# guptakhil/show-tell

Hardware: AMD Instinct MI355X
Metric: training images/sec (ResNet101+GRU, emb=512, bs=128) at 1/2/4/8 MI355X (higher is better)
Workload: dtype bf16; 1 GPU; BASELINE configs[1]: ResNet-101 (train-mode BN, frozen) + 5-layer GRU decoder, E=H=512, V=10000, fwd+bwd+SGD step, synthetic COCO-shaped batch; batch_per_gpu=128, global_batch=128, image=3x224x224, parallelism=dp1

## Files before the change

### include/showtell_hip.h

```cpp
#ifndef SHOWTELL_HIP_H
#define SHOWTELL_HIP_H

#include <stddef.h>
#include <stdint.h>

#ifdef __cplusplus
extern "C" {
#endif

#define ST_F32 0
#define ST_BF16 1

#define ST_CELL_GRU 0
#define ST_CELL_LSTM 1

const char* st_last_error(void);
int st_version(void);

typedef struct {
  const void* x;
  const void* w;
  void* y;
  const float* bias;
  const float* scale;
// ... 168 lines not shown

int st_cast2d(const void* x, void* y, int from_dtype, int to_dtype, int rows, int cols, int ldx, int ldy, void* stream);

#define ST_MAX_LAYERS 8
typedef struct {
  int cell, dtype, L, in0, H, V, E;
  const void* emb;
  const void* w_ih[ST_MAX_LAYERS]; const void* w_hh[ST_MAX_LAYERS];
  const float* b_ih[ST_MAX_LAYERS]; const float* b_hh[ST_MAX_LAYERS];
  const void* w_lin; const float* b_lin;
} st_rnn_params;

typedef struct {
  float* emb;
  float* w_ih[ST_MAX_LAYERS]; float* w_hh[ST_MAX_LAYERS]; float* b_ih[ST_MAX_LAYERS]; float* b_hh[ST_MAX_LAYERS];
  float* w_lin; float* b_lin;
} st_rnn_grads;

typedef struct {
  int B, T, ntok, Tcap;
  const int* batch_sizes_host;
  const int* rows_b; const int* rows_t; const int* prev_row;
  const long* caption;
} st_packed_seq;

int st_rnn_vocab_ld(int V);
size_t st_rnn_workspace_bytes(const st_rnn_params* p, const st_packed_seq* s);
int st_rnn_forward(const st_rnn_params* p, const st_packed_seq* s, const void* x0_override, const void* feat,
                   void* workspace, size_t workspace_bytes, void* logits, int logits_dtype, int ldl,
                   long* targets, int save_for_backward, void* stream);
int st_rnn_backward(const st_rnn_params* p, const st_rnn_grads* g, const st_packed_seq* s,
                    const void* x0_override, const void* dlogits, int ldd, const float* dy_top,
                    void* workspace, size_t workspace_bytes, float* dfeat, float* dx0_out, void* stream);

int st_rnn_fused_loss_supported(const st_rnn_params* p);
size_t st_rnn_fused_loss_bytes(const st_rnn_params* p, const st_packed_seq* s);
int st_rnn_fused_loss(const st_rnn_params* p, const st_packed_seq* s, const void* workspace, size_t workspace_bytes,
                      const long* targets, float* scratch, size_t scratch_bytes, float* loss_accum, void* stream);
int st_rnn_fused_dlogits(const st_rnn_params* p, const st_packed_seq* s, const void* workspace, size_t workspace_bytes,
                         const long* targets, const float* scratch, const float* grad_scale_dev, void* dlogits, int ldd, void* stream);

int st_cross_entropy(const void* logits, int logits_dtype, const long* target, int rows, int V, int ldl,
                     float* loss_accum, void* dlogits, int dlogits_dtype, int ldd, float grad_scale,
                     const float* grad_scale_dev , void* stream);

size_t st_head_workspace_bytes(int B, int F, int E, int dtype);
int st_linear_bn1d_forward(const void* x, const void* w, const float* bias, const float* gamma, const float* beta,
                           float* running_mean, float* running_var, int B, int F, int E, int dtype,
                           int train, float momentum, float eps,
                           float* z_out, float* save_mean, float* save_rstd, void* y_dtype, float* y_f32, void* stream);
int st_linear_bn1d_backward(const float* dy, const float* z, const void* x, const float* gamma,
                            const float* save_mean, const float* save_rstd, int B, int F, int E, int dtype, int train,
                            float* dw, float* dbias, float* dgamma, float* dbeta, void* workspace, size_t workspace_bytes,
                            void* stream);

int st_sgd_step(float* param, const float* grad, float* momentum_buf, void* bf16_shadow, long n,
                float lr, float momentum, int first_step, float grad_scale, void* stream);
int st_adam_step(float* param, const float* grad, float* exp_avg, float* exp_avg_sq, void* bf16_shadow, long n,
                 float lr, float beta1, float beta2, float eps, int step, float grad_scale, void* stream);

size_t st_rnn_greedy_workspace_bytes(const st_rnn_params* p, int B);
int st_rnn_greedy(const st_rnn_params* p, const void* feat, int B, int steps, void* workspace, size_t workspace_bytes,
                  long* ids_out, float* logits_out, void* stream);
int st_rnn_greedy_last_route(void);

int st_rnn_step(const st_rnn_params* p, const void* x, int n, const void* h_in, const void* c_in,
// ... 47 lines not shown
```

### show-tell_amd/_lib.py

```python
import ctypes as C
import os

_HERE = os.path.dirname(os.path.abspath(__file__))
LIB_PATH = os.path.join(_HERE, "lib", "libshowtell_hip.so")

ST_F32, ST_BF16 = 0, 1
ST_CELL_GRU, ST_CELL_LSTM = 0, 1

c_p, c_i, c_f, c_l = C.c_void_p, C.c_int, C.c_float, C.c_long


class ConvDesc(C.Structure):
    _fields_ = [("x", c_p), ("w", c_p), ("y", c_p), ("bias", c_p), ("scale", c_p), ("shift", c_p),
                ("residual", c_p), ("stats", c_p), ("dtype", c_i), ("out_dtype", c_i),
                ("B", c_i), ("Hin", c_i), ("Win", c_i), ("Cin", c_i), ("Ho", c_i), ("Wo", c_i), ("N", c_i),
                ("KH", c_i), ("KW", c_i), ("stride", c_i), ("pad", c_i),
                ("ldx", c_i), ("ldw", c_i), ("ldy", c_i), ("relu", c_i), ("accumulate", c_i), ("Cin_logical", c_i), ("k_order", c_i), ("stats_replicas", c_i),
                ("in_stats", c_p), ("in_gamma", c_p), ("in_beta", c_p), ("in_count", c_f), ("in_eps", c_f), ("split_k", c_i)]


class Conv3x3ImgDesc(C.Structure):
    _fields_ = [("x", c_p), ("w_frag", c_p), ("y", c_p), ("stats", c_p), ("stats_replicas", c_i), ("scale", c_p), ("shift", c_p),
                ("relu", c_i), ("in_stats", c_p), ("in_gamma", c_p), ("in_beta", c_p), ("in_count", c_f), ("in_eps", c_f),
                ("B", c_i), ("H", c_i), ("W", c_i), ("C", c_i), ("N", c_i), ("in_stats_replicas", c_i)]
# ... 103 lines not shown
    "st_conv1x1_kstream": ([C.POINTER(Conv1x1WregDesc), c_p], c_i),
    "st_pack_conv_weight_frag": ([c_p, c_p, c_i, c_i, c_i, c_i, c_i, c_p], c_i),
    "st_tune": ([c_i, c_i, c_i], c_i),
    "st_prof_enable": ([c_i], c_i),
    "st_debug_stamps": ([c_p], c_i),
    "st_prof_collect": ([C.POINTER(C.c_double), C.POINTER(C.c_double), C.POINTER(c_l)], c_i),
    "st_bn_act": ([C.POINTER(BnActDesc), c_p], c_i),
    "st_bn_update_running": ([c_p, c_p, c_p, c_i, c_f, c_f, c_p], c_i),
    "st_nchw_to_nhwc": ([c_p, c_p, c_i, c_i, c_i, c_i, c_i, c_i, c_p], c_i),
    "st_nchw_to_s2d16": ([c_p, c_p, c_i, c_i, c_i, c_i, c_p], c_i),
    "st_stem_weight_s2d": ([c_p, c_p, c_i, c_i, c_p], c_i),
    "st_stem_weight_frag": ([c_p, c_p, c_p], c_i),
    "st_stem_weight_frag_packed": ([c_p, c_i, c_p, c_p], c_i),
    "st_stem_conv_pool": ([C.POINTER(StemConvPoolDesc), c_p], c_i),
    "st_nhwc_to_ncp_f32": ([c_p, c_p, c_i, c_i, c_i, c_i, c_p], c_i),
    "st_maxpool3x3s2": ([c_p, c_p, c_i, c_i, c_i, c_i, c_i, c_p], c_i),
    "st_maxpool3x3s2_bn": ([c_p, c_p, c_i, c_i, c_i, c_i, c_i, c_p, c_p, c_p, c_p, c_p, c_f, c_f, c_p], c_i),
    "st_global_avgpool": ([c_p, c_p, c_i, c_i, c_i, c_i, c_i, c_p], c_i),
    "st_cast": ([c_p, c_p, c_i, c_i, c_l, c_p], c_i),
    "st_transpose": ([c_p, c_p, c_i, c_i, c_i, c_i, c_i, c_p], c_i),
    "st_transpose_colsum": ([c_p, c_p, c_p, c_i, c_i, c_i, c_i, c_i, c_p], c_i),
    "st_transpose_batch": ([c_p, c_p, c_p, c_i, c_i, c_i, c_i, c_i, c_i, c_p, c_p, c_p], c_i),
    "st_pack_conv_weight": ([c_p, c_p, c_i, c_i, c_i, c_i, c_i, c_i, c_i, c_p], c_i),
    "st_cast2d": ([c_p, c_p, c_i, c_i, c_i, c_i, c_i, c_i, c_p], c_i),
    "st_rnn_vocab_ld": ([c_i], c_i),
    "st_rnn_workspace_bytes": ([C.POINTER(RnnParams), C.POINTER(PackedSeq)], C.c_size_t),
    "st_rnn_forward": ([C.POINTER(RnnParams), C.POINTER(PackedSeq), c_p, c_p, c_p, C.c_size_t, c_p, c_i, c_i, c_p, c_i, c_p], c_i),
    "st_rnn_fused_loss_supported": ([C.POINTER(RnnParams)], c_i),
    "st_rnn_fused_loss_bytes": ([C.POINTER(RnnParams), C.POINTER(PackedSeq)], C.c_size_t),
    "st_rnn_fused_loss": ([C.POINTER(RnnParams), C.POINTER(PackedSeq), c_p, C.c_size_t, c_p, c_p, C.c_size_t, c_p, c_p], c_i),
    "st_rnn_fused_dlogits": ([C.POINTER(RnnParams), C.POINTER(PackedSeq), c_p, C.c_size_t, c_p, c_p, c_p, c_p, c_i, c_p], c_i),
    "st_rnn_backward": ([C.POINTER(RnnParams), C.POINTER(RnnGrads), C.POINTER(PackedSeq), c_p, c_p, c_i, c_p, c_p, C.c_size_t,
                         c_p, c_p, c_p], c_i),
    "st_rnn_greedy_workspace_bytes": ([C.POINTER(RnnParams), c_i], C.c_size_t),
    "st_rnn_greedy": ([C.POINTER(RnnParams), c_p, c_i, c_i, c_p, C.c_size_t, c_p, c_p, c_p], c_i),
    "st_rnn_greedy_last_route": ([], c_i),
    "st_rnn_step": ([C.POINTER(RnnParams), c_p, c_i, c_p, c_p, c_p, c_p, c_p, c_i, c_p], c_i),
    "st_embedding_rows": ([c_p, c_p, c_p, c_i, c_i, c_i, c_i, c_i, c_p], c_i),
    "st_gather_state": ([c_p, c_p, c_p, c_i, c_i, c_i, c_i, c_i, c_p], c_i),
    "st_softmax_topk": ([c_p, c_i, c_i, c_i, c_i, c_p, c_p, c_i, c_p], c_i),
    "st_beam_select": ([c_p, c_p, c_p, c_p, c_p, c_i, c_i, c_i, c_l, c_p, c_p, c_p, c_p, c_p, c_p], c_i),
    "st_attn_workspace_bytes": ([c_p, c_p], C.c_size_t),
    "st_attn_forward": ([c_p, c_p, c_p, c_p, c_p, C.c_size_t, c_p, c_i, c_i, c_p, c_i, c_p], c_i),
    "st_attn_backward": ([c_p, c_p, c_p, c_p, c_p, c_i, c_p, c_p, c_f, c_p, c_p, C.c_size_t, c_p], c_i),
    "st_attn_reg_loss": ([c_p, c_i, c_i, c_i, c_f, c_p, c_p], c_i),
    "st_attn_greedy_workspace_bytes": ([c_p, c_i], C.c_size_t),
    "st_attn_greedy": ([c_p, c_p, c_i, c_i, c_l, c_p, C.c_size_t, c_p, c_p], c_i),
    "st_attn_greedy_alphas": ([c_p, c_p, c_i, c_i, c_l, c_p, C.c_size_t, c_p, c_p, c_p], c_i),
    "st_attn_beam_workspace_bytes": ([c_p, c_i, c_i], C.c_size_t),
    "st_attn_beam_search": ([c_p, c_p, c_i, c_i, c_i, c_l, c_l, c_p, C.c_size_t, c_p, c_p, c_p, c_p, c_p, c_p], c_i),
    "st_cross_entropy": ([c_p, c_i, c_p, c_i, c_i, c_i, c_p, c_p, c_i, c_i, c_f, c_p, c_p], c_i),
    "st_head_workspace_bytes": ([c_i, c_i, c_i, c_i], C.c_size_t),
    "st_linear_bn1d_forward": ([c_p] * 7 + [c_i, c_i, c_i, c_i, c_i, c_f, c_f] + [c_p] * 6, c_i),
    "st_linear_bn1d_backward": ([c_p] * 6 + [c_i, c_i, c_i, c_i, c_i] + [c_p] * 5 + [C.c_size_t, c_p], c_i),
    "st_sgd_step": ([c_p, c_p, c_p, c_p, c_l, c_f, c_f, c_i, c_f, c_p], c_i),
    "st_adam_step": ([c_p, c_p, c_p, c_p, c_p, c_l, c_f, c_f, c_f, c_f, c_i, c_f, c_p], c_i),
    "st_resnet_create": ([c_i, c_i, C.POINTER(c_p)], c_i),
    "st_resnet_destroy": ([c_p], None),
    "st_resnet_num_convs": ([c_p], c_i),
    "st_resnet_feat_dim": ([c_p], c_i),
    "st_resnet_weight_elems": ([c_p], C.c_size_t),
    "st_resnet_bn_channels": ([c_p], C.c_size_t),
    "st_resnet_conv_info": ([c_p, c_i] + [C.POINTER(c_i)] * 6 + [C.POINTER(C.c_size_t)] * 2 + [C.POINTER(c_i), C.POINTER(C.c_size_t), C.POINTER(c_i)], c_i),
    "st_resnet_workspace_bytes": ([c_p, c_i, c_i, c_i], C.c_size_t),
    "st_resnet_set_taps": ([c_p, c_p, C.c_size_t], c_i),
    "st_resnet_forward": ([c_p, c_p, c_i, c_i, c_i, c_p, c_p, c_p, c_p, c_p, c_i, c_f, c_f, c_p, C.c_size_t,
# ... 47 lines not shown
```

### show-tell_amd/csrc/rnn.cpp

```cpp
#include "common.h"
#include "rnn_kernels.h"
#include <string.h>
#include <vector>

namespace {

inline size_t al(size_t v) { return (v + 255) & ~(size_t)255; }
inline int up8(int v) { return (v + 7) & ~7; }

struct Plan {
  int G, GH, Np, Vp, maxw;
  size_t es;
  size_t x0, y, gates, cst, dyl, dx0, dgx, dgh, dhc, dcc, tA, tB, wT, wThh, wTih, gA, gB, total;
};

Plan make_plan(const st_rnn_params* p, const st_packed_seq* s) {
  Plan q;
  q.G = p->cell == ST_CELL_GRU ? 3 : 4;
  q.GH = q.G * p->H;
  q.Np = up8(s->ntok);
  q.Vp = st_rnn_vocab_ld(p->V);
  q.es = st_dtype_size(p->dtype);
  q.maxw = p->in0 > p->H ? p->in0 : p->H;
  const size_t n = s->ntok, L = p->L, H = p->H;
  size_t o = 0;
  auto take = [&](size_t bytes) { size_t r = o; o += al(bytes); return r; };
  q.x0 = take(n * p->in0 * q.es);
  q.y = take(L * n * H * q.es);
  q.gates = take(L * n * 4 * H * q.es);
  q.cst = take(p->cell == ST_CELL_LSTM ? L * n * H * q.es : 0);
  q.dyl = take(L * n * H * sizeof(float));
  q.dx0 = take(n * p->in0 * sizeof(float));
  q.dgx = take(L * n * q.GH * q.es);
  q.dgh = take(p->cell == ST_CELL_GRU ? L * n * q.GH * q.es : 0);
// ... 113 lines not shown
}

extern "C" int st_rnn_fused_loss_supported(const st_rnn_params* p) {
  return p && p->w_lin && p->b_lin && vocab_ce_supported(p->dtype, p->H) ? 1 : 0;
}
extern "C" size_t st_rnn_fused_loss_bytes(const st_rnn_params* p, const st_packed_seq* s) {
  if (!p || !s) return 0;
  return ((size_t)s->ntok * (2 + 2 * (size_t)vocab_ce_tiles(p->V))) * sizeof(float);
}
extern "C" int st_rnn_fused_loss(const st_rnn_params* p, const st_packed_seq* s, const void* workspace, size_t workspace_bytes,
                                 const long* targets, float* scratch, size_t scratch_bytes, float* loss_accum, void* stream) {
  if (check_common(p, s, "st_rnn_fused_loss")) return 1;
  ST_CHECK(workspace && targets && scratch && loss_accum, "st_rnn_fused_loss: null pointer");
  ST_CHECK(st_rnn_fused_loss_supported(p), "st_rnn_fused_loss: needs bf16, H = 512 and the vocabulary projection (use st_rnn_forward's logits + st_cross_entropy)");
  const Plan q = make_plan(p, s);
  ST_CHECK(workspace_bytes >= q.total && scratch_bytes >= st_rnn_fused_loss_bytes(p, s), "st_rnn_fused_loss: workspace / scratch too small");
  const char* ytop = reinterpret_cast<const char*>(workspace) + q.y + (size_t)(p->L - 1) * s->ntok * p->H * q.es;
  const int n = s->ntok;
  return vocab_ce_forward(ytop, p->w_lin, p->b_lin, targets, n, p->V, scratch + 2 * (size_t)n, scratch + n, scratch, loss_accum,
                          reinterpret_cast<hipStream_t>(stream));
}
extern "C" int st_rnn_fused_dlogits(const st_rnn_params* p, const st_packed_seq* s, const void* workspace, size_t workspace_bytes,
                                    const long* targets, const float* scratch, const float* grad_scale_dev, void* dlogits, int ldd, void* stream) {
  if (check_common(p, s, "st_rnn_fused_dlogits")) return 1;
  ST_CHECK(workspace && targets && scratch && dlogits, "st_rnn_fused_dlogits: null pointer");
  ST_CHECK(st_rnn_fused_loss_supported(p), "st_rnn_fused_dlogits: unsupported configuration");
  const Plan q = make_plan(p, s);
  ST_CHECK(workspace_bytes >= q.total, "st_rnn_fused_dlogits: workspace too small");
  const char* ytop = reinterpret_cast<const char*>(workspace) + q.y + (size_t)(p->L - 1) * s->ntok * p->H * q.es;
  return vocab_ce_dlogits(ytop, p->w_lin, p->b_lin, targets, scratch, s->ntok, p->V, dlogits, ldd, 1.0f, grad_scale_dev,
                          reinterpret_cast<hipStream_t>(stream));
}

extern "C" int st_rnn_backward(const st_rnn_params* p, const st_rnn_grads* g, const st_packed_seq* s,
                               const void* x0_override, const void* dlogits, int ldd, const float* dy_top_extra,
                               void* workspace, size_t workspace_bytes, float* dfeat, float* dx0_out, void* stream) {
  if (check_common(p, s, "st_rnn_backward")) return 1;
  ST_CHECK(g && workspace, "st_rnn_backward: null pointer");
  const Plan q = make_plan(p, s);
  ST_CHECK(workspace_bytes >= q.total, "st_rnn_backward: workspace too small (%zu < %zu)", workspace_bytes, q.total);
  hipStream_t st = reinterpret_cast<hipStream_t>(stream);
  char* ws = reinterpret_cast<char*>(workspace);
  const int dt = p->dtype, H = p->H, n = s->ntok, Np = q.Np, GH = q.GH;
  const size_t es = q.es;
  std::vector<int> off(s->T + 1, 0);
  for (int t = 0; t < s->T; ++t) off[t + 1] = off[t] + s->batch_sizes_host[t];
  const int L = p->L, T = s->T;
  auto dyl = [&](int l) { return reinterpret_cast<float*>(ws + q.dyl) + (size_t)l * n * H; };
  float* dy = dyl(L - 1);
  const char* ytop = ws + q.y + (size_t)(p->L - 1) * n * H * es;

  if (dlogits) {
    ST_CHECK(p->w_lin && g->w_lin && g->b_lin, "st_rnn_backward: vocabulary projection gradients requested without buffers");
    ST_CHECK(ldd >= up8(p->V) && ldd % 8 == 0 && ldd <= q.Vp, "st_rnn_backward: dlogits leading dimension %d must be a multiple of 8 in [%d, %d]",
             ldd, up8(p->V), q.Vp);
    if (st_transpose_colsum(dlogits, ws + q.tA, g->b_lin, dt, n, p->V, ldd, Np, stream)) return 1;
    if (st_transpose(ytop, ws + q.tB, dt, n, H, H, Np, stream)) return 1;
    if (gemm_nt(ws + q.tA, Np, ws + q.tB, Np, g->w_lin, H, p->V, H, Np, dt, ST_F32, nullptr, 1, stream)) return 1;
    if (st_transpose(p->w_lin, ws + q.wT, dt, p->V, H, H, ldd, stream)) return 1;
    const int bk = dt == ST_BF16 ? 64 : 32;
    const int split = (ldd % (8 * bk) == 0 && ldd >= 16 * bk) ? 8 : 0;
    if (gemm_nt(dlogits, ldd, ws + q.wT, ldd, dy, H, n, H, ldd, dt, ST_F32, nullptr, 0, stream, split)) return 1;
    if (dy_top_extra) { st_set_error("st_rnn_backward: dlogits and dy_top_extra are exclusive"); return 1; }
  } else {
    ST_CHECK(dy_top_extra, "st_rnn_backward: need dlogits or dy_top");
    if (hipMemcpyAsync(dy, dy_top_extra, (size_t)n * H * sizeof(float), hipMemcpyDeviceToDevice, st) != hipSuccess) {
      st_set_error("st_rnn_backward: copy failed"); return 1;
    }
  }

  const void* x0 = x0_override ? x0_override : ws + q.x0;
  const bool need_dx0 = dfeat || dx0_out || g->emb;
  float* dx0 = dx0_out ? dx0_out : reinterpret_cast<float*>(ws + q.dx0);
  const bool gru = p->cell == ST_CELL_GRU;
  auto dgxl = [&](int l) { return ws + q.dgx + (size_t)l * n * GH * es; };
  auto dghl = [&](int l) { return gru ? ws + q.dgh + (size_t)l * n * GH * es : dgxl(l); };
  auto dhcl = [&](int l) { return reinterpret_cast<float*>(ws + q.dhc) + (size_t)l * s->B * H; };
  auto dccl = [&](int l) { return reinterpret_cast<float*>(ws + q.dcc) + (size_t)l * s->B * H; };
  auto wThh = [&](int l) { return ws + q.wThh + (size_t)l * H * GH * es; };
  auto wTih = [&](int l) { return ws + q.wTih + (size_t)l * q.maxw * GH * es; };
  if (hipMemsetAsync(ws + q.dhc, 0, (size_t)L * s->B * H * sizeof(float), st) != hipSuccess ||
      hipMemsetAsync(ws + q.dcc, 0, (size_t)L * s->B * H * sizeof(float), st) != hipSuccess) { st_set_error("memset failed"); return 1; }
  {
    const void* wx[2][ST_MAX_LAYERS]; void* wy[2][ST_MAX_LAYERS];
    int ni = 0;
    for (int l = 0; l < L; ++l) {
      const int in = l == 0 ? p->in0 : H;
      wx[0][l] = p->w_hh[l]; wy[0][l] = wThh(l);
      if (!(l > 0 || need_dx0)) continue;
      if (in == H) { wx[1][ni] = p->w_ih[l]; wy[1][ni] = wTih(l); ++ni; }
      else if (st_transpose(p->w_ih[l], wTih(l), dt, GH, in, in, GH, stream)) return 1;
    }
    if (st_transpose_batch(wx[0], wy[0], nullptr, L, dt, GH, H, H, GH, nullptr, nullptr, stream)) return 1;
    if (ni && st_transpose_batch(wx[1], wy[1], nullptr, ni, dt, GH, H, H, GH, nullptr, nullptr, stream)) return 1;
  }
  for (int d = T + L - 2; d >= 0; --d) {
    RnnBwdCell gc[ST_MAX_LAYERS];
    RnnGemmArgs mc[2 * ST_MAX_LAYERS];
    int ng = 0, nm = 0;
    for (int l = d < T ? 0 : d - (T - 1); l <= d && l < L; ++l) {
      const int t = d - l;
      const int bt = s->batch_sizes_host[t];
      const int in = l == 0 ? p->in0 : H;
      char* yl = ws + q.y + (size_t)l * n * H * es;
      char* gl = ws + q.gates + (size_t)l * n * 4 * H * es;
      char* cl = ws + q.cst + (size_t)l * n * H * es;
      RnnBwdCell& c = gc[ng++];
      memset(&c, 0, sizeof(c));
      c.dy = dyl(l) + (size_t)off[t] * H; c.dhc = dhcl(l); c.dcc = dccl(l);
      c.cache = gl + (size_t)off[t] * 4 * H * es;
      c.hprev = t > 0 ? yl + (size_t)off[t - 1] * H * es : nullptr;
      c.cnew = cl + (size_t)off[t] * H * es;
      c.cprev = t > 0 ? cl + (size_t)off[t - 1] * H * es : nullptr;
      c.dgx = dgxl(l) + (size_t)off[t] * GH * es; c.dgh = dghl(l) + (size_t)off[t] * GH * es; c.Bt = bt;
      if (t > 0) {
        RnnGemmArgs& a = mc[nm++];
        memset(&a, 0, sizeof(a));
        a.A = dghl(l) + (size_t)off[t] * GH * es; a.W = wThh(l); a.M = bt; a.N = H; a.K = GH; a.lda = GH; a.ldw = GH;
        a.out_f32 = dhcl(l); a.ldo = H; a.accumulate = 1;
      }
      if (l > 0 || need_dx0) {
        RnnGemmArgs& a = mc[nm++];
        memset(&a, 0, sizeof(a));
        a.A = dgxl(l) + (size_t)off[t] * GH * es; a.W = wTih(l); a.M = bt; a.N = in; a.K = GH; a.lda = GH; a.ldw = GH;
        a.out_f32 = (l > 0 ? dyl(l - 1) + (size_t)off[t] * H : dx0 + (size_t)off[t] * in); a.ldo = in;
      }
    }
    if (rnn_bwd_gates_launch_batch(gc, ng, H, p->cell, dt, st)) return 1;
    if (rnn_gemm_launch_batch(mc, nm, dt, 0, 0, st)) return 1;
// ... 50 lines not shown
```

### show-tell_amd/csrc/rnn_kernels.h

```cpp
#pragma once
#include "common.h"

struct RnnGemmArgs {
  const void* A; const void* W; int M, N, K, lda, ldw, gstride;
  const void* A2; const void* W2; int K2, lda2, ldw2;
  float* out_f32; int ldo; int accumulate;
  const float* bias_h; const float* bias_x;
  const void* gx; int ldgx;
  const void* hprev; const void* cprev; int ldhp;
  void* hout; void* cout; int ldho;
  void* hout2; int ldho2;
  void* cache; int ldcache;
  unsigned long long* argmax_keys;
  const unsigned long long* x_keys; int x_V;
  long* ids_out; int ids_stride, ids_t;
};
constexpr int kCellRawOut = 1, kCellSplit = 2;

constexpr int kRnnBatch = 16;
struct RnnGemmBatch { RnnGemmArgs c[kRnnBatch]; };
static_assert(sizeof(RnnGemmBatch) <= 4000, "kernel-argument segment is 4 KiB");
struct RnnBwdCell {
  const float* dy; float* dhc; float* dcc; const void* cache; const void* hprev; const void* cnew; const void* cprev;
  void* dgx; void* dgh; int Bt;
};
struct RnnBwdBatch { RnnBwdCell c[kRnnBatch]; };

#ifdef __HIPCC__
__device__ __forceinline__ float st_sigm(float x) { return 1.0f / (1.0f + expf(-x)); }
__device__ __forceinline__ float st_gru_unit(float xr, float xz, float xn, float hr, float hz, float hn, float hprev, float& r, float& z, float& n) {
  r = st_sigm(xr + hr);
  z = st_sigm(xz + hz);
  n = tanhf(__builtin_fmaf(r, hn, xn));
  return __builtin_fmaf(z, hprev, (1.f - z) * n);
}
__device__ __forceinline__ float st_lstm_unit(float pi, float pf, float pg, float po, float cprev, float& ig, float& fg, float& gg, float& og, float& cn) {
  ig = st_sigm(pi); fg = st_sigm(pf); gg = tanhf(pg); og = st_sigm(po);
  cn = __builtin_fmaf(fg, cprev, ig * gg);
  return og * tanhf(cn);
}
#endif

size_t rnn_greedy_pipe_bytes(const st_rnn_params* p, int B, int steps);
int rnn_greedy_pipe(const st_rnn_params* p, const void* feat, int B, int steps, void* ws, size_t ws_bytes, long* ids_out, hipStream_t st);

int vocab_ce_supported(int dtype, int H);
int vocab_ce_tiles(int V);
int vocab_ce_forward(const void* y, const void* w, const float* bias, const long* target, int n, int V, float* partial, float* tgt,
                     float* lse, float* loss, hipStream_t st);
int vocab_ce_dlogits(const void* y, const void* w, const float* bias, const long* target, const float* lse, int n, int V,
                     void* dlogits, int ldd, float gscale, const float* gscale_dev, hipStream_t st);

int rnn_gemm_launch(const RnnGemmArgs& a, int dtype, int epi, int has_x, hipStream_t st);
int rnn_gemm_launch_batch(const RnnGemmArgs* cells, int ncells, int dtype, int epi, int has_x, hipStream_t st);
int rnn_bwd_gates_launch_batch(const RnnBwdCell* cells, int ncells, int H, int cell_kind, int dtype, hipStream_t st);
int pack_inputs_launch(const void* feat, const void* emb, const long* cap, int Tcap, const int* rows_b, const int* rows_t,
                       void* x0, long* target, int ntok, int E, int V, int mode, int dtype, hipStream_t st);
int embedding_bwd_launch(const float* dx0, const long* cap, int Tcap, const int* rows_b, const int* rows_t,
                         float* dfeat, float* demb, int ntok, int E, int V, int mode, hipStream_t st);
int gather_hprev_launch(const void* y, const int* rows_t, const int* prev_row, void* hp, int ntok, int H, int dtype, hipStream_t st,
                        const void* h0 = nullptr, const int* rows_b = nullptr);
int gru_bwd_gates_launch(const float* dy, float* dhc, const void* cache, const void* hprev, void* dgx, void* dgh,
                         int Bt, int H, int dtype, hipStream_t st);
int lstm_bwd_gates_launch(const float* dy, float* dhc, float* dcc, const void* cache, const void* cnew, const void* cprev,
                          void* dg, int Bt, int H, int dtype, hipStream_t st);
int colsum_launch(const void* x, float* out, int rows, int cols, int ldx, int dtype, hipStream_t st);
```

### show-tell_amd/csrc/rnn_kernels.hip

```cpp
#include "common.h"
#include "rnn_kernels.h"
#include <string.h>

namespace {

template <typename T> struct Mfma;
template <> struct Mfma<bf16_t> {
  static constexpr int EPC = 8;
  static __device__ __forceinline__ void run(const u32x4& a, const u32x4& b, f32x4& c) {
    c = __builtin_amdgcn_mfma_f32_16x16x32_bf16(*reinterpret_cast<const bf16x8*>(&a),
                                                *reinterpret_cast<const bf16x8*>(&b), c, 0, 0, 0);
  }
};
template <> struct Mfma<float> {
  static constexpr int EPC = 4;
  static __device__ __forceinline__ void run(const u32x4& a, const u32x4& b, f32x4& c) {
#pragma unroll
    for (int e = 0; e < 4; ++e)
      c = __builtin_amdgcn_mfma_f32_16x16x4f32(__uint_as_float(a[e]), __uint_as_float(b[e]), c, 0, 0, 0);
  }
};

template <typename T> __device__ __forceinline__ void load4(const T* p, float* v);
template <> __device__ __forceinline__ void load4<float>(const float* p, float* v) {
// ... 283 lines not shown
                                                           const T* __restrict__ h0, const int* __restrict__ rows_b) {
  constexpr int N = 16 / (int)sizeof(T);
  const int cpr = H / N;
  const long total = (long)ntok * cpr;
  for (long i = (long)blockIdx.x * blockDim.x + threadIdx.x; i < total; i += (long)gridDim.x * blockDim.x) {
    const int row = (int)(i / cpr), c = (int)(i - (long)row * cpr) * N;
    u32x4 v = {0u, 0u, 0u, 0u};
    if (rows_t[row] > 0) v = *reinterpret_cast<const u32x4*>(y + (long)prev_row[row] * H + c);
    else if (h0) v = *reinterpret_cast<const u32x4*>(h0 + (long)rows_b[row] * H + c);
    *reinterpret_cast<u32x4*>(hp + (long)row * H + c) = v;
  }
}

template <typename T>
__global__ __launch_bounds__(256) void gru_bwd_gates_kernel(RnnBwdBatch batch, int H) {
  const RnnBwdCell& cl = batch.c[blockIdx.y];
  const float* __restrict__ dy = cl.dy; float* __restrict__ dhc = cl.dhc;
  const T* __restrict__ cache = reinterpret_cast<const T*>(cl.cache);
  const T* __restrict__ hprev = reinterpret_cast<const T*>(cl.hprev);
  T* __restrict__ dgx = reinterpret_cast<T*>(cl.dgx); T* __restrict__ dgh = reinterpret_cast<T*>(cl.dgh);
  const int Bt = cl.Bt;
  const int total = Bt * (H / 4);
  const int i = blockIdx.x * blockDim.x + threadIdx.x;
  if (i >= total) return;
  const int b = i / (H / 4), j = (i - b * (H / 4)) * 4;
  float g[4], c[4], r[4], z[4], n[4], hn[4], hp[4] = {0.f, 0.f, 0.f, 0.f};
  load4<float>(dy + (long)b * H + j, g);
  load4<float>(dhc + (long)b * H + j, c);
  const T* cr = cache + (long)b * 4 * H + j;
  load4<T>(cr, r); load4<T>(cr + H, z); load4<T>(cr + 2 * H, n); load4<T>(cr + 3 * H, hn);
  if (hprev) load4<T>(hprev + (long)b * H + j, hp);
  float drp[4], dzp[4], dnp[4], dnr[4], dhz[4];
#pragma unroll
  for (int e = 0; e < 4; ++e) {
    const float dh = g[e] + c[e];
    const float dn = dh * (1.f - z[e]);
    const float dz = dh * (hp[e] - n[e]);
    dnp[e] = dn * (1.f - n[e] * n[e]);
    drp[e] = dnp[e] * hn[e] * r[e] * (1.f - r[e]);
    dzp[e] = dz * z[e] * (1.f - z[e]);
    dnr[e] = dnp[e] * r[e];
    dhz[e] = dh * z[e];
  }
  T* ox = dgx + (long)b * 3 * H + j;
  T* oh = dgh + (long)b * 3 * H + j;
  store4<T>(ox, drp); store4<T>(ox + H, dzp); store4<T>(ox + 2 * H, dnp);
  store4<T>(oh, drp); store4<T>(oh + H, dzp); store4<T>(oh + 2 * H, dnr);
  store4<float>(dhc + (long)b * H + j, dhz);
}

template <typename T>
__global__ __launch_bounds__(256) void lstm_bwd_gates_kernel(RnnBwdBatch batch, int H) {
  const RnnBwdCell& cl = batch.c[blockIdx.y];
  const float* __restrict__ dy = cl.dy; float* __restrict__ dhc = cl.dhc; float* __restrict__ dcc = cl.dcc;
  const T* __restrict__ cache = reinterpret_cast<const T*>(cl.cache);
  const T* __restrict__ cnew = reinterpret_cast<const T*>(cl.cnew);
  const T* __restrict__ cprev = reinterpret_cast<const T*>(cl.cprev);
  T* __restrict__ dg = reinterpret_cast<T*>(cl.dgx);
  const int Bt = cl.Bt;
  const int total = Bt * (H / 4);
  const int i = blockIdx.x * blockDim.x + threadIdx.x;
  if (i >= total) return;
  const int b = i / (H / 4), j = (i - b * (H / 4)) * 4;
  float g[4], ch[4], cc[4], ig[4], fg[4], gg[4], og[4], cn[4], cp[4] = {0.f, 0.f, 0.f, 0.f};
  load4<float>(dy + (long)b * H + j, g);
  load4<float>(dhc + (long)b * H + j, ch);
  load4<float>(dcc + (long)b * H + j, cc);
  const T* cr = cache + (long)b * 4 * H + j;
  load4<T>(cr, ig); load4<T>(cr + H, fg); load4<T>(cr + 2 * H, gg); load4<T>(cr + 3 * H, og);
  load4<T>(cnew + (long)b * H + j, cn);
  if (cprev) load4<T>(cprev + (long)b * H + j, cp);
  float di[4], df[4], dgg[4], dob[4], dcp[4], zero[4] = {0.f, 0.f, 0.f, 0.f};
#pragma unroll
  for (int e = 0; e < 4; ++e) {
    const float dh = g[e] + ch[e];
    const float tc = tanhf(cn[e]);
    const float dc = cc[e] + dh * og[e] * (1.f - tc * tc);
    dob[e] = dh * tc * og[e] * (1.f - og[e]);
    di[e] = dc * gg[e] * ig[e] * (1.f - ig[e]);
    df[e] = dc * cp[e] * fg[e] * (1.f - fg[e]);
    dgg[e] = dc * ig[e] * (1.f - gg[e] * gg[e]);
    dcp[e] = dc * fg[e];
  }
  T* o = dg + (long)b * 4 * H + j;
  store4<T>(o, di); store4<T>(o + H, df); store4<T>(o + 2 * H, dgg); store4<T>(o + 3 * H, dob);
  store4<float>(dcc + (long)b * H + j, dcp);
  store4<float>(dhc + (long)b * H + j, zero);
}

template <typename TL, typename TD>
__global__ __launch_bounds__(256) void ce_kernel(const TL* __restrict__ logits, const long* __restrict__ target,
                                                 float* __restrict__ loss, TD* __restrict__ dlogits,
                                                 int V, int ldl, int ldd, float inv_rows, float gscale, const float* __restrict__ gscale_dev) {
  __shared__ float sm[8], ss[8];
  const int row = blockIdx.x;
  const TL* x = logits + (long)row * ldl;
  float m = -INFINITY, s = 0.f;
  for (int i = threadIdx.x; i < V; i += blockDim.x) {
    const float v = to_f32<TL>(x[i]);
    const float nm = fmaxf(m, v);
    s = s * __expf(m - nm) + __expf(v - nm);
    m = nm;
  }
#pragma unroll
  for (int o = 32; o > 0; o >>= 1) {
    const float om = __shfl_xor(m, o, 64), os = __shfl_xor(s, o, 64);
    const float nm = fmaxf(m, om);
    s = (m == -INFINITY ? 0.f : s * __expf(m - nm)) + (om == -INFINITY ? 0.f : os * __expf(om - nm));
    m = nm;
  }
  const int lane = threadIdx.x & 63, wid = threadIdx.x >> 6;
  if (lane == 0) { sm[wid] = m; ss[wid] = s; }
  __syncthreads();
  float M = sm[0], S = ss[0];
  for (int w = 1; w < (int)(blockDim.x >> 6); ++w) {
    const float nm = fmaxf(M, sm[w]);
// ... 181 lines not shown
```

Measured before the change: 31770 images/sec.

## Fuse RNN backward recurrent GEMMs with gate-gradient epilogue in one MFMA kernel

Adds a bf16 MFMA kernel that computes, per wavefront diagonal, the recurrent dh GEMM (dgh_next·W_hh^T) and the upper-layer dx GEMM (dgx_up·W_ih^T), reduces them across waves in LDS, and applies the GRU/LSTM backward gate math in the epilogue. This replaces the separate GEMM launches and the gates kernel for each diagonal step, and also removes the carry-buffer memsets. It is on by default and can be disabled with ST_RNN_BWD_FUSED=0. The dx0 GEMM is moved to one batched launch after the loop. The kernel uses small 32x32 tiles with K split across 4 waves, which may underuse the MFMA units compared with the tuned GEMM path.

```diff
diff --git a/include/showtell_hip.h b/include/showtell_hip.h
--- a/include/showtell_hip.h
+++ b/include/showtell_hip.h
@@ -224,6 +224,7 @@
 int st_rnn_backward(const st_rnn_params* p, const st_rnn_grads* g, const st_packed_seq* s,
                     const void* x0_override, const void* dlogits, int ldd, const float* dy_top,
                     void* workspace, size_t workspace_bytes, float* dfeat, float* dx0_out, void* stream);
+int st_rnn_backward_last_route(void);
 
 int st_rnn_fused_loss_supported(const st_rnn_params* p);
 size_t st_rnn_fused_loss_bytes(const st_rnn_params* p, const st_packed_seq* s);
diff --git a/show-tell_amd/_lib.py b/show-tell_amd/_lib.py
--- a/show-tell_amd/_lib.py
+++ b/show-tell_amd/_lib.py
@@ -159,6 +159,7 @@
     "st_rnn_fused_dlogits": ([C.POINTER(RnnParams), C.POINTER(PackedSeq), c_p, C.c_size_t, c_p, c_p, c_p, c_p, c_i, c_p], c_i),
     "st_rnn_backward": ([C.POINTER(RnnParams), C.POINTER(RnnGrads), C.POINTER(PackedSeq), c_p, c_p, c_i, c_p, c_p, C.c_size_t,
                          c_p, c_p, c_p], c_i),
+    "st_rnn_backward_last_route": ([], c_i),
     "st_rnn_greedy_workspace_bytes": ([C.POINTER(RnnParams), c_i], C.c_size_t),
     "st_rnn_greedy": ([C.POINTER(RnnParams), c_p, c_i, c_i, c_p, C.c_size_t, c_p, c_p, c_p], c_i),
     "st_rnn_greedy_last_route": ([], c_i),
diff --git a/show-tell_amd/csrc/rnn.cpp b/show-tell_amd/csrc/rnn.cpp
--- a/show-tell_amd/csrc/rnn.cpp
+++ b/show-tell_amd/csrc/rnn.cpp
@@ -1,5 +1,7 @@
 #include "common.h"
 #include "rnn_kernels.h"
+#include <atomic>
+#include <stdlib.h>
 #include <string.h>
 #include <vector>
 
@@ -179,9 +181,14 @@
                           reinterpret_cast<hipStream_t>(stream));
 }
 
+static std::atomic<int> g_bwd_route{1};
+
+extern "C" int st_rnn_backward_last_route(void) { return g_bwd_route; }
+
 extern "C" int st_rnn_backward(const st_rnn_params* p, const st_rnn_grads* g, const st_packed_seq* s,
                                const void* x0_override, const void* dlogits, int ldd, const float* dy_top_extra,
                                void* workspace, size_t workspace_bytes, float* dfeat, float* dx0_out, void* stream) {
+  g_bwd_route = 1;
   if (check_common(p, s, "st_rnn_backward")) return 1;
   ST_CHECK(g && workspace, "st_rnn_backward: null pointer");
   const Plan q = make_plan(p, s);
@@ -226,8 +233,13 @@
   auto dccl = [&](int l) { return reinterpret_cast<float*>(ws + q.dcc) + (size_t)l * s->B * H; };
   auto wThh = [&](int l) { return ws + q.wThh + (size_t)l * H * GH * es; };
   auto wTih = [&](int l) { return ws + q.wTih + (size_t)l * q.maxw * GH * es; };
-  if (hipMemsetAsync(ws + q.dhc, 0, (size_t)L * s->B * H * sizeof(float), st) != hipSuccess ||
-      hipMemsetAsync(ws + q.dcc, 0, (size_t)L * s->B * H * sizeof(float), st) != hipSuccess) { st_set_error("memset failed"); return 1; }
+  const char* env = getenv("ST_RNN_BWD_FUSED");
+  const bool fused = (!env || atoi(env) != 0) && rnn_bwd_fused_supported(dt, H, L);
+  g_bwd_route = fused ? 0 : 1;
+  if (!fused && (hipMemsetAsync(ws + q.dhc, 0, (size_t)L * s->B * H * sizeof(float), st) != hipSuccess ||
+                 hipMemsetAsync(ws + q.dcc, 0, (size_t)L * s->B * H * sizeof(float), st) != hipSuccess)) {
+    st_set_error("memset failed"); return 1;
+  }
   {
     const void* wx[2][ST_MAX_LAYERS]; void* wy[2][ST_MAX_LAYERS];
     int ni = 0;
@@ -241,7 +253,39 @@
     if (st_transpose_batch(wx[0], wy[0], nullptr, L, dt, GH, H, H, GH, nullptr, nullptr, stream)) return 1;
     if (ni && st_transpose_batch(wx[1], wy[1], nullptr, ni, dt, GH, H, H, GH, nullptr, nullptr, stream)) return 1;
   }
-  for (int d = T + L - 2; d >= 0; --d) {
+  for (int d = T + L - 2; fused && d >= 0; --d) {
+    RnnBwdFusedCell fc[ST_MAX_LAYERS];
+    int nf = 0;
+    for (int l = d < T ? 0 : d - (T - 1); l <= d && l < L; ++l) {
+      const int t = d - l;
+      RnnBwdFusedCell& c = fc[nf++];
+      memset(&c, 0, sizeof(c));
+      c.Bt = s->batch_sizes_host[t];
+      c.Bn = t + 1 < T ? s->batch_sizes_host[t + 1] : 0;
+      c.dgh_next = t + 1 < T ? dghl(l) + (size_t)off[t + 1] * GH * es : nullptr;
+      c.w_hh_t = wThh(l);
+      if (l + 1 < L) { c.dgx_up = dgxl(l + 1) + (size_t)off[t] * GH * es; c.w_ih_up_t = wTih(l + 1); }
+      else c.dy_top = dy + (size_t)off[t] * H;
+      const char* yl = ws + q.y + (size_t)l * n * H * es;
+      const char* cl = ws + q.cst + (size_t)l * n * H * es;
+      c.cache = ws + q.gates + (size_t)l * n * 4 * H * es + (size_t)off[t] * 4 * H * es;
+      c.hprev = gru && t > 0 ? yl + (size_t)off[t - 1] * H * es : nullptr;
+      c.cnew = gru ? nullptr : cl + (size_t)off[t] * H * es;
+      c.cprev = !gru && t > 0 ? cl + (size_t)off[t - 1] * H * es : nullptr;
+      c.dgx = dgxl(l) + (size_t)off[t] * GH * es;
+      c.dgh = gru ? dghl(l) + (size_t)off[t] * GH * es : nullptr;
+      c.carry = gru ? dhcl(l) : dccl(l);
+    }
+    if (rnn_bwd_fused_launch_batch(fc, nf, H, p->cell, st)) return 1;
+  }
+  if (fused && need_dx0) {
+    RnnGemmArgs a;
+    memset(&a, 0, sizeof(a));
+    a.A = dgxl(0); a.W = wTih(0); a.M = n; a.N = p->in0; a.K = GH; a.lda = GH; a.ldw = GH;
+    a.out_f32 = dx0; a.ldo = p->in0;
+    if (rnn_gemm_launch_batch(&a, 1, dt, 0, 0, st)) return 1;
+  }
+  for (int d = T + L - 2; !fused && d >= 0; --d) {
     RnnBwdCell gc[ST_MAX_LAYERS];
     RnnGemmArgs mc[2 * ST_MAX_LAYERS];
     int ng = 0, nm = 0;
diff --git a/show-tell_amd/csrc/rnn_bwd_fused.hip b/show-tell_amd/csrc/rnn_bwd_fused.hip
--- /dev/null
+++ b/show-tell_amd/csrc/rnn_bwd_fused.hip
@@ -0,0 +1,190 @@
+#include "common.h"
+#include "rnn_kernels.h"
+#include <string.h>
+
+namespace {
+
+constexpr int kRows = 32, kUnits = 32;
+constexpr int MT = kRows / 16, NT = kUnits / 16;
+static_assert(MT >= 1 && MT <= 4, "wave w < MT runs the epilogue of row tile w");
+constexpr int UNR = 4;
+
+__device__ __forceinline__ void unpack4(const u32x2 t, float* v) {
+  v[0] = __uint_as_float(t[0] << 16); v[1] = __uint_as_float(t[0] & 0xffff0000u);
+  v[2] = __uint_as_float(t[1] << 16); v[3] = __uint_as_float(t[1] & 0xffff0000u);
+}
+__device__ __forceinline__ void store4_bf16(bf16_t* p, const float* v) {
+  *reinterpret_cast<u32x2*>(p) = u32x2{pack_bf16x2(v[0], v[1]), pack_bf16x2(v[2], v[3])};
+}
+__device__ __forceinline__ void mfma(const u32x4& a, const u32x4& b, f32x4& c) {
+  c = __builtin_amdgcn_mfma_f32_16x16x32_bf16(*reinterpret_cast<const bf16x8*>(&a), *reinterpret_cast<const bf16x8*>(&b), c, 0, 0, 0);
+}
+
+__device__ __forceinline__ void reduce_waves(f32x4 (&red)[4][MT][NT][64], const f32x4 (&acc)[MT][NT], f32x4 (&sum)[NT],
+                                             int wid, int lane) {
+#pragma unroll
+  for (int t = 0; t < MT; ++t)
+#pragma unroll
+    for (int u = 0; u < NT; ++u) red[wid][t][u][lane] = acc[t][u];
+  __syncthreads();
+#pragma unroll
+  for (int u = 0; u < NT; ++u) {
+    if (wid >= MT) break;
+    sum[u] = red[0][wid][u][lane];
+#pragma unroll
+    for (int w = 1; w < 4; ++w) sum[u] += red[w][wid][u][lane];
+  }
+  __syncthreads();
+}
+
+template <int NG>
+__global__ __launch_bounds__(256) void rnn_bwd_fused_kernel(RnnBwdFusedBatch batch, int H) {
+  const RnnBwdFusedCell& c = batch.c[blockIdx.z];
+  __shared__ f32x4 red[4][MT][NT][64];
+  const int lane = threadIdx.x & 63;
+  const int wid = __builtin_amdgcn_readfirstlane(threadIdx.x >> 6);
+  const int r16 = lane & 15, q4 = lane >> 4;
+  const int n0 = blockIdx.x * kUnits, mbase = blockIdx.y * kRows;
+  if (mbase >= c.Bt) return;
+  const int K = NG * H;
+  const bool has1 = c.dgh_next && mbase < c.Bn, has2 = c.dgx_up != nullptr;
+  const int m = mbase + wid * 16 + r16;
+  const bool live = wid < MT && m < c.Bt, carried = m < c.Bn;
+
+  f32x4 acc1[MT][NT], acc2[MT][NT];
+#pragma unroll
+  for (int t = 0; t < MT; ++t)
+#pragma unroll
+    for (int u = 0; u < NT; ++u) { acc1[t][u] = f32x4{0.f, 0.f, 0.f, 0.f}; acc2[t][u] = f32x4{0.f, 0.f, 0.f, 0.f}; }
+  const bf16_t* A1[MT]; const bf16_t* A2[MT]; bool ok1[MT], ok2[MT];
+#pragma unroll
+  for (int t = 0; t < MT; ++t) {
+    const int mm = mbase + 16 * t + r16;
+    ok1[t] = has1 && mm < c.Bn;
+    ok2[t] = has2 && mm < c.Bt;
+    A1[t] = reinterpret_cast<const bf16_t*>(c.dgh_next) + (long)mm * K;
+    A2[t] = reinterpret_cast<const bf16_t*>(c.dgx_up) + (long)mm * K;
+  }
+  const bf16_t* W1 = reinterpret_cast<const bf16_t*>(c.w_hh_t) + (long)(n0 + r16) * K;
+  const bf16_t* W2 = reinterpret_cast<const bf16_t*>(c.w_ih_up_t) + (long)(n0 + r16) * K;
+  const int ns = K / 32, spw = (ns + 3) / 4, beg = wid * spw, end = min(ns, beg + spw);
+  for (int s0 = beg; s0 < end; s0 += UNR) {
+    u32x4 fa1[MT][UNR], fw1[UNR][NT], fa2[MT][UNR], fw2[UNR][NT];
+#pragma unroll
+    for (int v = 0; v < UNR; ++v) {
+      const bool ok = s0 + v < end;
+      const int k = ((s0 + v) * 4 + q4) * 8;
+#pragma unroll
+      for (int t = 0; t < MT; ++t) {
+        fa1[t][v] = u32x4{0u, 0u, 0u, 0u}; fa2[t][v] = u32x4{0u, 0u, 0u, 0u};
+        if (ok && ok1[t]) fa1[t][v] = *reinterpret_cast<const u32x4*>(A1[t] + k);
+        if (ok && ok2[t]) fa2[t][v] = *reinterpret_cast<const u32x4*>(A2[t] + k);
+      }
+#pragma unroll
+      for (int u = 0; u < NT; ++u) {
+        fw1[v][u] = u32x4{0u, 0u, 0u, 0u}; fw2[v][u] = u32x4{0u, 0u, 0u, 0u};
+        if (ok && has1) fw1[v][u] = *reinterpret_cast<const u32x4*>(W1 + (long)u * 16 * K + k);
+        if (ok && has2) fw2[v][u] = *reinterpret_cast<const u32x4*>(W2 + (long)u * 16 * K + k);
+      }
+    }
+    if (has1) {
+#pragma unroll
+      for (int v = 0; v < UNR; ++v)
+#pragma unroll
+        for (int u = 0; u < NT; ++u)
+#pragma unroll
+          for (int t = 0; t < MT; ++t) mfma(fw1[v][u], fa1[t][v], acc1[t][u]);
+    }
+    if (has2) {
+#pragma unroll
+      for (int v = 0; v < UNR; ++v)
+#pragma unroll
+        for (int u = 0; u < NT; ++u)
+#pragma unroll
+          for (int t = 0; t < MT; ++t) mfma(fw2[v][u], fa2[t][v], acc2[t][u]);
+    }
+  }
+  u32x2 ca[NT][4], hp[NT], cn[NT];
+  f32x4 cy[NT], dy[NT];
+#pragma unroll
+  for (int u = 0; u < NT; ++u) {
+    const int n = n0 + 16 * u + 4 * q4;
+#pragma unroll
+    for (int g = 0; g < 4; ++g) ca[u][g] = u32x2{0u, 0u};
+    hp[u] = u32x2{0u, 0u}; cn[u] = u32x2{0u, 0u};
+    cy[u] = f32x4{0.f, 0.f, 0.f, 0.f}; dy[u] = f32x4{0.f, 0.f, 0.f, 0.f};
+    if (!live) continue;
+    const bf16_t* cr = reinterpret_cast<const bf16_t*>(c.cache) + (long)m * 4 * H + n;
+#pragma unroll
+    for (int g = 0; g < 4; ++g) ca[u][g] = *reinterpret_cast<const u32x2*>(cr + g * H);
+    const void* prev = NG == 3 ? c.hprev : c.cprev;
+    if (prev) hp[u] = *reinterpret_cast<const u32x2*>(reinterpret_cast<const bf16_t*>(prev) + (long)m * H + n);
+    if (NG == 4) cn[u] = *reinterpret_cast<const u32x2*>(reinterpret_cast<const bf16_t*>(c.cnew) + (long)m * H + n);
+    if (carried) cy[u] = *reinterpret_cast<const f32x4*>(c.carry + (long)m * H + n);
+    if (!has2) dy[u] = *reinterpret_cast<const f32x4*>(c.dy_top + (long)m * H + n);
+  }
+
+  f32x4 s1[NT], s2[NT];
+#pragma unroll
+  for (int u = 0; u < NT; ++u) { s1[u] = f32x4{0.f, 0.f, 0.f, 0.f}; s2[u] = dy[u]; }
+  if (has1) reduce_waves(red, acc1, s1, wid, lane);
+  if (has2) reduce_waves(red, acc2, s2, wid, lane);
+  if (!live) return;
+
+#pragma unroll
+  for (int u = 0; u < NT; ++u) {
+    const int n = n0 + 16 * u + 4 * q4;
+    float g0[4], g1[4], g2[4], g3[4], pv[4], cv[4], o0[4], o1[4], o2[4], o3[4], cr[4];
+    unpack4(ca[u][0], g0); unpack4(ca[u][1], g1); unpack4(ca[u][2], g2); unpack4(ca[u][3], g3);
+    unpack4(hp[u], pv); unpack4(cn[u], cv);
+    bf16_t* ox = reinterpret_cast<bf16_t*>(c.dgx) + (long)m * K + n;
+    if (NG == 3) {
+#pragma unroll
+      for (int e = 0; e < 4; ++e) {
+        const float dh = s2[u][e] + (carried ? s1[u][e] + cy[u][e] : 0.f);
+        st_gru_bwd_unit(dh, g0[e], g1[e], g2[e], g3[e], pv[e], o0[e], o1[e], o2[e], o3[e], cr[e]);
+      }
+      bf16_t* oh = reinterpret_cast<bf16_t*>(c.dgh) + (long)m * K + n;
+      store4_bf16(ox, o0); store4_bf16(ox + H, o1); store4_bf16(ox + 2 * H, o2);
+      store4_bf16(oh, o0); store4_bf16(oh + H, o1); store4_bf16(oh + 2 * H, o3);
+    } else {
+#pragma unroll
+      for (int e = 0; e < 4; ++e) {
+        const float dh = s2[u][e] + (carried ? s1[u][e] : 0.f);
+        st_lstm_bwd_unit(dh, carried ? cy[u][e] : 0.f, g0[e], g1[e], g2[e], g3[e], cv[e], pv[e], o0[e], o1[e], o2[e], o3[e], cr[e]);
+      }
+      store4_bf16(ox, o0); store4_bf16(ox + H, o1); store4_bf16(ox + 2 * H, o2); store4_bf16(ox + 3 * H, o3);
+    }
+    *reinterpret_cast<f32x4*>(c.carry + (long)m * H + n) = f32x4{cr[0], cr[1], cr[2], cr[3]};
+  }
+}
+
+}
+
+int rnn_bwd_fused_supported(int dtype, int H, int L) {
+  return dtype == ST_BF16 && H > 0 && H % kUnits == 0 && L >= 1 && L <= kRnnBatch ? 1 : 0;
+}
+
+int rnn_bwd_fused_launch_batch(const RnnBwdFusedCell* cells, int ncells, int H, int cell_kind, hipStream_t st) {
+  ST_CHECK(ncells >= 0 && ncells <= kRnnBatch, "rnn_bwd_fused: %d cells in one launch (max %d)", ncells, kRnnBatch);
+  ST_CHECK(H > 0 && H % kUnits == 0, "rnn_bwd_fused: H=%d must be a multiple of %d", H, kUnits);
+  ST_CHECK(cell_kind == ST_CELL_GRU || cell_kind == ST_CELL_LSTM, "rnn_bwd_fused: bad cell %d", cell_kind);
+  RnnBwdFusedBatch b;
+  memset(&b, 0, sizeof(b));
+  int nc = 0, maxB = 0;
+  for (int i = 0; i < ncells; ++i) {
+    const RnnBwdFusedCell& c = cells[i];
+    if (c.Bt <= 0) continue;
+    ST_CHECK(c.Bn >= 0 && c.Bn <= c.Bt && (c.Bn == 0 || c.dgh_next) && (c.dgx_up ? c.w_ih_up_t != nullptr : c.dy_top != nullptr) &&
+             c.w_hh_t && c.cache && c.dgx && c.carry && (cell_kind == ST_CELL_LSTM ? c.cnew != nullptr : c.dgh != nullptr),
+             "rnn_bwd_fused: bad cell descriptor %d", i);
+    b.c[nc++] = c;
+    if (c.Bt > maxB) maxB = c.Bt;
+  }
+  if (nc == 0) return 0;
+  const dim3 grid(H / kUnits, (maxB + kRows - 1) / kRows, nc), block(256);
+  if (cell_kind == ST_CELL_GRU) hipLaunchKernelGGL(rnn_bwd_fused_kernel<3>, grid, block, 0, st, b, H);
+  else hipLaunchKernelGGL(rnn_bwd_fused_kernel<4>, grid, block, 0, st, b, H);
+  ST_LAUNCH_CHECK();
+  return 0;
+}
diff --git a/show-tell_amd/csrc/rnn_kernels.h b/show-tell_amd/csrc/rnn_kernels.h
--- a/show-tell_amd/csrc/rnn_kernels.h
+++ b/show-tell_amd/csrc/rnn_kernels.h
@@ -25,6 +25,17 @@
   void* dgx; void* dgh; int Bt;
 };
 struct RnnBwdBatch { RnnBwdCell c[kRnnBatch]; };
+struct RnnBwdFusedCell {
+  const void* dgh_next; const void* w_hh_t;
+  const void* dgx_up; const void* w_ih_up_t;
+  const float* dy_top;
+  const void* cache; const void* hprev; const void* cnew; const void* cprev;
+  void* dgx; void* dgh;
+  float* carry;
+  int Bt, Bn;
+};
+struct RnnBwdFusedBatch { RnnBwdFusedCell c[kRnnBatch]; };
+static_assert(sizeof(RnnBwdFusedBatch) <= 4000, "kernel-argument segment is 4 KiB");
 
 #ifdef __HIPCC__
 __device__ __forceinline__ float st_sigm(float x) { return 1.0f / (1.0f + expf(-x)); }
@@ -38,6 +49,28 @@
   ig = st_sigm(pi); fg = st_sigm(pf); gg = tanhf(pg); og = st_sigm(po);
   cn = __builtin_fmaf(fg, cprev, ig * gg);
   return og * tanhf(cn);
+}
+__device__ __forceinline__ void st_gru_bwd_unit(float dh, float r, float z, float n, float hn, float hprev,
+                                                float& drp, float& dzp, float& dnp, float& dnr, float& dhz) {
+#pragma clang fp contract(off)
+  const float dn = dh * (1.f - z);
+  const float dz = dh * (hprev - n);
+  dnp = dn * __builtin_fmaf(-n, n, 1.f);
+  drp = dnp * hn * r * (1.f - r);
+  dzp = dz * z * (1.f - z);
+  dnr = dnp * r;
+  dhz = dh * z;
+}
+__device__ __forceinline__ void st_lstm_bwd_unit(float dh, float dcc, float ig, float fg, float gg, float og, float cn, float cprev,
+                                                 float& di, float& df, float& dgg, float& dob, float& dcp) {
+#pragma clang fp contract(off)
+  const float tc = tanhf(cn);
+  const float dc = __builtin_fmaf(dh * og, __builtin_fmaf(-tc, tc, 1.f), dcc);
+  dob = dh * tc * og * (1.f - og);
+  di = dc * gg * ig * (1.f - ig);
+  df = dc * cprev * fg * (1.f - fg);
+  dgg = dc * ig * __builtin_fmaf(-gg, gg, 1.f);
+  dcp = dc * fg;
 }
 #endif
 
@@ -54,6 +87,8 @@
 int rnn_gemm_launch(const RnnGemmArgs& a, int dtype, int epi, int has_x, hipStream_t st);
 int rnn_gemm_launch_batch(const RnnGemmArgs* cells, int ncells, int dtype, int epi, int has_x, hipStream_t st);
 int rnn_bwd_gates_launch_batch(const RnnBwdCell* cells, int ncells, int H, int cell_kind, int dtype, hipStream_t st);
+int rnn_bwd_fused_supported(int dtype, int H, int L);
+int rnn_bwd_fused_launch_batch(const RnnBwdFusedCell* cells, int ncells, int H, int cell_kind, hipStream_t st);
 int pack_inputs_launch(const void* feat, const void* emb, const long* cap, int Tcap, const int* rows_b, const int* rows_t,
                        void* x0, long* target, int ntok, int E, int V, int mode, int dtype, hipStream_t st);
 int embedding_bwd_launch(const float* dx0, const long* cap, int Tcap, const int* rows_b, const int* rows_t,
diff --git a/show-tell_amd/csrc/rnn_kernels.hip b/show-tell_amd/csrc/rnn_kernels.hip
--- a/show-tell_amd/csrc/rnn_kernels.hip
+++ b/show-tell_amd/csrc/rnn_kernels.hip
@@ -339,16 +339,7 @@
   if (hprev) load4<T>(hprev + (long)b * H + j, hp);
   float drp[4], dzp[4], dnp[4], dnr[4], dhz[4];
 #pragma unroll
-  for (int e = 0; e < 4; ++e) {
-    const float dh = g[e] + c[e];
-    const float dn = dh * (1.f - z[e]);
-    const float dz = dh * (hp[e] - n[e]);
-    dnp[e] = dn * (1.f - n[e] * n[e]);
-    drp[e] = dnp[e] * hn[e] * r[e] * (1.f - r[e]);
-    dzp[e] = dz * z[e] * (1.f - z[e]);
-    dnr[e] = dnp[e] * r[e];
-    dhz[e] = dh * z[e];
-  }
+  for (int e = 0; e < 4; ++e) st_gru_bwd_unit(g[e] + c[e], r[e], z[e], n[e], hn[e], hp[e], drp[e], dzp[e], dnp[e], dnr[e], dhz[e]);
   T* ox = dgx + (long)b * 3 * H + j;
   T* oh = dgh + (long)b * 3 * H + j;
   store4<T>(ox, drp); store4<T>(ox + H, dzp); store4<T>(ox + 2 * H, dnp);
@@ -379,16 +370,7 @@
   if (cprev) load4<T>(cprev + (long)b * H + j, cp);
   float di[4], df[4], dgg[4], dob[4], dcp[4], zero[4] = {0.f, 0.f, 0.f, 0.f};
 #pragma unroll
-  for (int e = 0; e < 4; ++e) {
-    const float dh = g[e] + ch[e];
-    const float tc = tanhf(cn[e]);
-    const float dc = cc[e] + dh * og[e] * (1.f - tc * tc);
-    dob[e] = dh * tc * og[e] * (1.f - og[e]);
-    di[e] = dc * gg[e] * ig[e] * (1.f - ig[e]);
-    df[e] = dc * cp[e] * fg[e] * (1.f - fg[e]);
-    dgg[e] = dc * ig[e] * (1.f - gg[e] * gg[e]);
-    dcp[e] = dc * fg[e];
-  }
+  for (int e = 0; e < 4; ++e) st_lstm_bwd_unit(g[e] + ch[e], cc[e], ig[e], fg[e], gg[e], og[e], cn[e], cp[e], di[e], df[e], dgg[e], dob[e], dcp[e]);
   T* o = dg + (long)b * 4 * H + j;
   store4<T>(o, di); store4<T>(o + H, df); store4<T>(o + 2 * H, dgg); store4<T>(o + 3 * H, dob);
   store4<float>(dcc + (long)b * H + j, dcp);
```

Measured after the change: 31980 images/sec (median of 6 runs). About the same (+0.7%).
